# bghira/SimpleTuner

Measured on AMD Instinct MI355X. Metric: training images/sec (whole node), Flux.1-dev LoRA r32 1024^2 train step, higher is better.
Workload: dtype bf16

## Files before the change

### simpletuner_amd/csrc/gemm.hip

```cpp
#include <stdlib.h>
#include <type_traits>
#include "common.h"

#define BK 64
#define EPI_SPLITK 100

#ifdef ST355_TRACE
#define TR_T0 40
#define TR_MARKS 12
__device__ uint64_t st355_trace_buf[2][TR_MARKS];
#define TR_DECL uint64_t tr_[TR_MARKS] = {}
#define TR(t, k)                                                  \
  do {                                                            \
    if ((t) == TR_T0) tr_[k] = __builtin_amdgcn_s_memtime();       \
  } while (0)
#define TR_FLUSH(wv, lane)                                                              \
  do {                                                                                  \
    if (blockIdx.x == 64 && (lane) == 0 && ((wv) & 3) == 0)                              \
      for (int k_ = 0; k_ < TR_MARKS; k_++) st355_trace_buf[(wv) >> 2][k_] = tr_[k_];    \
  } while (0)
#else
#define TR_DECL
#define TR(t, k)
#define TR_FLUSH(wv, lane)
#endif

struct GemmP {
  const bf16* A; int64_t lda;
  const bf16* B; int64_t ldb;
  const bf16* A2; int64_t lda2;
  const bf16* B2; int64_t ldb2;
  bf16* C; int64_t ldc;
  int M, N, K, K2;
  const bf16* bias;
  bf16* aux_out; int64_t ld_aux_out;
  const bf16* aux_in; int64_t ld_aux_in;
  const bf16* gate; int64_t gate_stride; int64_t rows_per_batch;
  float* partial; int ksplit;
  int64_t part_ld;
  const float* scale_a; const float* scale_b;
  int conv_taps, conv_tpt, conv_wp, conv_hp;
  int skip_dead = 1;
  int64_t conv_row0;
  const bf16* img_add; int64_t img_add_stride;
  int seg_rows = 0;
  int64_t seg_xa = 0, seg_xa2 = 0, seg_xc = 0, seg_xin = 0, seg_xout = 0;
  uint32_t tn_magic = 0; int tn_skip_a = 0, tn_skip_b = 0;
  bf16* rq = nullptr; bf16* rk = nullptr; float* rrms = nullptr; bf16* rvt = nullptr; int rSp = 0;
  const bf16* rwq = nullptr; const bf16* rwk = nullptr;
  const float* rcos = nullptr; const float* rsin = nullptr;
  int rH = 0, rS = 0, rpos0 = 0;
  float reps = 0.f;
  int hq = 0, hk = 0;
};

__device__ __forceinline__ GemmP seg_view(const GemmP& p0, int m0) {
  GemmP p = p0;
  if (p0.seg_rows) {
// ... 535 lines not shown
        }
      }
    }
  }
}

__device__ __forceinline__ bool epl_aligned(const GemmP& p) {
  bool ok = (p.N % 8 == 0) && (p.ldc % 8 == 0) && (((uintptr_t)p.C & 15) == 0);
  if (p.bias) ok = ok && (((uintptr_t)p.bias & 15) == 0);
  if (p.aux_out) ok = ok && (p.ld_aux_out % 8 == 0) && (((uintptr_t)p.aux_out & 15) == 0);
  if (p.aux_in) ok = ok && (p.ld_aux_in % 8 == 0) && (((uintptr_t)p.aux_in & 15) == 0);
  if (p.gate) ok = ok && (p.gate_stride % 8 == 0) && (((uintptr_t)p.gate & 15) == 0);
  if (p.img_add) ok = ok && (p.img_add_stride % 8 == 0) && (((uintptr_t)p.img_add & 15) == 0);
  return ok;
}

__device__ __forceinline__ void mma_tile(const char* xs, const char* ws, const int (&x_off)[2], const int (&x_sw)[2],
                                         const int (&w_off)[2], const int (&w_sw)[2], int khalf, f32x16 (&acc)[2][2]) {
#pragma unroll
  for (int ks = 0; ks < 4; ks++) {
    const int c = 2 * ks + khalf;
    bf16x8 wf[2], xf[2];
#pragma unroll
    for (int i = 0; i < 2; i++) {
      wf[i] = *(const bf16x8*)(ws + w_off[i] + ((c ^ w_sw[i]) << 4));
      xf[i] = *(const bf16x8*)(xs + x_off[i] + ((c ^ x_sw[i]) << 4));
    }
#pragma unroll
    for (int i = 0; i < 2; i++)
#pragma unroll
      for (int j = 0; j < 2; j++) acc[i][j] = __builtin_amdgcn_mfma_f32_32x32x16_bf16(wf[i], xf[j], acc[i][j], 0, 0, 0);
  }
}

#define P3_BM 256
#define P3_BN 128
#define P3_THREADS 512
#define P3_XBYTES (P3_BM * BK * 2)
#define P3_WBYTES (P3_BN * BK * 2)
#define P3_STAGE (P3_XBYTES + P3_WBYTES)
#define P3_LDS (3 * P3_STAGE)

template <int EPI>
__global__ void __launch_bounds__(P3_THREADS, 2) k_gemm_p3(GemmGroup g) {
  extern __shared__ __attribute__((aligned(16))) char smem[];
  const int tid = threadIdx.x;
  const int lane = tid & 63;
  const int wv = __builtin_amdgcn_readfirstlane(tid >> 6);
  const int wm = wv >> 1, wn = wv & 1;

  int id = xcd_remap(blockIdx.x, gridDim.x);
  const int pi = id >= g.tiles0 ? 1 : 0;
  if (pi) id -= g.tiles0;
  const GemmP& p0 = g.p[pi];
  const int nbm = (p0.M + P3_BM - 1) / P3_BM, nbn = (p0.N + P3_BN - 1) / P3_BN;
  int pm, pn;
  tile_coords(id, nbm, nbn, pm, pn);
  const int m0 = pm * P3_BM, n0 = pn * P3_BN;
  const GemmP p = seg_view(p0, m0);
  const int nt1 = p.K / BK;
  const int nt = nt1 + p.K2 / BK;

  const bf16* A1 = p.A; const bf16* B1 = p.B; const bf16* A2 = p.A2; const bf16* B2 = p.B2;
  const int64_t la2 = p.lda2, lb2 = p.ldb2;
  const int M = p.M, N = p.N;
  const int st_row = lane >> 3, st_cp = lane & 7;
// ... 2 lines not shown
#pragma unroll
  for (int j = 0; j < 4; j++) {
    const int row = (wv * 4 + j) * 8 + st_row;
    xc[j] = (st_cp ^ ((row >> 1) & 7)) * 8;
    xrow[j] = min(m0 + row, M - 1);
    xo[j] = (int64_t)xrow[j] * p.lda + xc[j];
  }
#pragma unroll
  for (int j = 0; j < 2; j++) {
    const int row = (wv * 2 + j) * 8 + st_row;
    wc[j] = (st_cp ^ ((row >> 1) & 7)) * 8;
    wrow[j] = min(n0 + row, N - 1);
    wo[j] = (int64_t)wrow[j] * p.ldb + wc[j];
  }
  auto stage = [&](int t, int buf) {
    char* xs = smem + buf * P3_STAGE;
    char* ws = xs + P3_XBYTES;
    if (t < nt1) {
      const int k0 = t * BK;
#pragma unroll
      for (int j = 0; j < 4; j++) glds16(A1 + xo[j] + k0, xs + (wv * 4 + j) * 1024);
#pragma unroll
      for (int j = 0; j < 2; j++) glds16(B1 + wo[j] + k0, ws + (wv * 2 + j) * 1024);
    } else {
      const int k0 = (t - nt1) * BK;
#pragma unroll
      for (int j = 0; j < 4; j++) glds16(A2 + (int64_t)xrow[j] * la2 + xc[j] + k0, xs + (wv * 4 + j) * 1024);
#pragma unroll
      for (int j = 0; j < 2; j++) glds16(B2 + (int64_t)wrow[j] * lb2 + wc[j] + k0, ws + (wv * 2 + j) * 1024);
    }
  };

  int w_off[2], w_sw[2], x_off[2], x_sw[2];
#pragma unroll
  for (int i = 0; i < 2; i++) {
    const int wr = wn * 64 + i * 32 + (lane & 31);
    w_off[i] = wr * 128; w_sw[i] = (wr >> 1) & 7;
    const int xr = wm * 64 + i * 32 + (lane & 31);
    x_off[i] = xr * 128; x_sw[i] = (xr >> 1) & 7;
  }
  const int khalf = lane >> 5;
  f32x16 acc[2][2];
#pragma unroll
  for (int i = 0; i < 2; i++)
#pragma unroll
    for (int j = 0; j < 2; j++)
#pragma unroll
      for (int r = 0; r < 16; r++) acc[i][j][r] = 0.f;

  stage(0, 0);
  if (nt > 1) {
    stage(1, 1);
    asm volatile("s_waitcnt vmcnt(6)" ::: "memory");
  } else {
    asm volatile("s_waitcnt vmcnt(0)" ::: "memory");
  }
  __builtin_amdgcn_s_barrier();
  int cur = 0;
  for (int t = 0; t < nt; t++) {
    if (t + 2 < nt) stage(t + 2, cur == 0 ? 2 : cur - 1);
    const char* xs = smem + cur * P3_STAGE;
    mma_tile(xs, xs + P3_XBYTES, x_off, x_sw, w_off, w_sw, khalf, acc);
    if (t + 1 < nt) {
      if (t + 2 < nt) asm volatile("s_waitcnt vmcnt(6)" ::: "memory");
      else asm volatile("s_waitcnt vmcnt(0)" ::: "memory");
      asm volatile("s_waitcnt lgkmcnt(0)" ::: "memory");
      __builtin_amdgcn_s_barrier();
    }
    cur = (cur == 2) ? 0 : cur + 1;
  }
  gemm_epilogue<EPI>(p, acc, m0 + wm * 64, n0 + wn * 64, lane);
}

#define PP_BARRIER()                                   \
  do {                                                 \
    asm volatile("" ::: "memory");                     \
    __builtin_amdgcn_s_barrier();                      \
    asm volatile("" ::: "memory");                     \
  } while (0)

#define PQ_BM 256
#define PQ_BN 256
#define PQ_BK 64
#define PQ_THREADS 512
#define PQ_REGION 16384
#define PQ_BUF (4 * PQ_REGION)
#define PQ_LDS (8 * 64 * 272)
#ifndef PQ_BUFLD
#define PQ_BUFLD 1
#endif
#ifndef PQ_VM
#define PQ_VM 8
#endif
#ifndef PQ_ABL
#define PQ_ABL 0
#endif
#ifndef PQ_PRIO
#ifndef PQ_F8_MX
#define PQ_F8_MX 1
#endif
typedef int i32x8 __attribute__((ext_vector_type(8)));
__device__ __forceinline__ i32x8 frag32(const long* p) {
  i32x8 v;
#pragma unroll
  for (int q = 0; q < 4; q++) { v[2 * q] = (int)(p[q] & 0xffffffffl); v[2 * q + 1] = (int)(p[q] >> 32); }
  return v;
}
#define PQ_PRIO 1
#endif
#ifndef PQ_GL
#define PQ_GL 1
#endif

__device__ __forceinline__ void wait_vm_rt(int n) {
  if (n >= 8) asm volatile("s_waitcnt vmcnt(8)" ::: "memory");
  else if (n == 6) asm volatile("s_waitcnt vmcnt(6)" ::: "memory");
  else if (n == 4) asm volatile("s_waitcnt vmcnt(4)" ::: "memory");
  else if (n == 2) asm volatile("s_waitcnt vmcnt(2)" ::: "memory");
  else asm volatile("s_waitcnt vmcnt(0)" ::: "memory");
}

template <int EPI, bool TN, bool F8 = false, bool CONV = false, int SK = 0>
__global__ void __launch_bounds__(PQ_THREADS, 2) k_gemm_pq(GemmGroup g) {
  static_assert(!SK || (!TN && !F8 && !CONV && EPI != EPI_SPLITK), "the stream-K tail is built for the plain NT bf16 problems");
  constexpr int ES = F8 ? 1 : 2;
  constexpr int KSN = F8 ? 8 : 4;
  static_assert(!(F8 && TN), "fp8 weight gradients are not built");
  extern __shared__ __attribute__((aligned(16))) char smem[];
  const int tid = threadIdx.x;
  const int lane = tid & 63;
  const int wv = __builtin_amdgcn_readfirstlane(tid >> 6);
  const int wm = wv >> 2, wn = wv & 3;

  int slice = (EPI == EPI_SPLITK) ? blockIdx.x / g.tiles0 : 0;
  int id = (EPI == EPI_SPLITK) ? xcd_remap(blockIdx.x % g.tiles0, g.tiles0) : xcd_remap(blockIdx.x, SK ? min((int)gridDim.x, g.sk_first) : (int)gridDim.x);
  int sk_n = 1, sk_tl = 0;
  if (SK && (int)blockIdx.x >= g.sk_first) {
    const int l = blockIdx.x - g.sk_first;
    sk_n = SK;
    const int lq = __builtin_amdgcn_readfirstlane((l >> 3) / sk_n);
    slice = (l >> 3) - lq * sk_n;
    sk_tl = 8 * lq + (l & 7);
    if (sk_tl >= g.tiles0 - g.sk_first) return;
    id = g.sk_first + sk_tl;
  }
  const int pi = id >= g.tiles0 ? 1 : 0;
  if (pi) id -= g.tiles0;
  const GemmP& p = g.p[pi];
  const int nbm = (p.M + PQ_BM - 1) / PQ_BM, nbn = (p.N + PQ_BN - 1) / PQ_BN;
  const int wtaps = (TN && p.conv_taps == 9) ? 9 : 1;
  int pm, pn;
  tile_coords(id, nbm, nbn * wtaps, pm, pn, TN ? ST355_TILE_GROUP : tile_group_for(p.K + p.K2));
  const int wtap = pn / nbn;
  pn -= wtap * nbn;
  const int m0 = pm * PQ_BM, n0 = pn * PQ_BN;
  const int64_t segi = (!TN && !F8 && !CONV && p.seg_rows) ? __builtin_amdgcn_readfirstlane(m0 / p.seg_rows) : 0;
  const int nt_all = p.K / (PQ_BK * 2 / ES);
  const int per = (EPI == EPI_SPLITK) ? (nt_all + p.ksplit - 1) / p.ksplit : SK ? __builtin_amdgcn_readfirstlane((nt_all + sk_n - 1) / sk_n) : nt_all;
  const int t_first = slice * per;
  const int nt1 = (EPI == EPI_SPLITK || SK) ? max(0, min(nt_all, t_first + per) - t_first) : nt_all;
  const int nt = nt1 + ((EPI == EPI_SPLITK || (SK && slice != sk_n - 1)) ? 0 : p.K2 / PQ_BK);
// ... 65 lines not shown
      stage_ext(A2, la2, m0, true, r, (u - nt1) * PQ_BK, dst);
    }
  };
  auto stage_w = [&](int u, int r) {
    char* dst = smem + (u & 1) * PQ_BUF + (2 + r) * PQ_REGION + wv * 2048;
    if (u < nt1) {
      const int w_ko = (int)(u * wk_step) + (TN ? (int)__umulhi((uint32_t)(u + t_first), p.tn_magic) * p.tn_skip_b : 0);
      if (PQ_BUFLD) {
#pragma unroll
        for (int j = 0; j < 2; j++)
          __builtin_amdgcn_raw_ptr_buffer_load_lds(w_rsrc, (__attribute__((address_space(3))) void*)(dst + j * 1024), 16, wo[r][j], w_ko, 0, 0);
        return;
      }
      const char* kb = wbase + w_ko;
#pragma unroll
      for (int j = 0; j < 2; j++) glds16((const bf16*)(kb + wo[r][j]), dst + j * 1024);
    } else {
      stage_ext(B2, lb2, n0, false, r, (u - nt1) * PQ_BK, dst);
    }
  };
  auto refill = [&](int t, int ph, bool check) {
    if (PQ_ABL & 2) return;
    if (ph == 0) { if (!check || t + 1 < nt) stage_w(t + 1, 1); }
    else if (ph == 1) { if (!check || t + 1 < nt) stage_x(t + 1, 1); }
    else if (ph == 2) { if (!check || t + 2 < nt) stage_x(t + 2, 0); }
    else { if (!check || t + 2 < nt) stage_w(t + 2, 0); }
  };

  const int khalf = lane >> 5;
  const int l31 = lane & 31;
  int xk[4], wk[4];
#pragma unroll
  for (int ks = 0; ks < 4; ks++) {
    const int ch = ((2 * ks + khalf) ^ ((l31 >> 1) & 7)) << 4;
    xk[ks] = (wm * 64 + l31) * 128 + ch;
    wk[ks] = 2 * PQ_REGION + (wn * 32 + l31) * 128 + ch;
  }
  const int tg = lane >> 4, tti = (lane >> 2) & 3, tts = lane & 3;
  const int t_row = (8 * (tg >> 1) + tti) * 256 + (tts & 1) * 8;
  const int xt = t_row + (((wm * 8 + 2 * (tg & 1) + (tts >> 1)) ^ (tti << 2)) << 4);
  const int wt = 2 * PQ_REGION + t_row + (((wn * 4 + 2 * (tg & 1) + (tts >> 1)) ^ (tti << 2)) << 4);
  int xk8[8], wk8[8];
#pragma unroll
  for (int ks = 0; ks < 8; ks++) {
    const int chunk = PQ_F8_MX ? 4 * (ks >> 2) + 2 * khalf + ((ks & 3) >> 1) : ks;
    const int half8 = PQ_F8_MX ? (ks & 1) : khalf;
    const int ch = ((chunk ^ ((l31 >> 1) & 7)) << 4) + half8 * 8;
    xk8[ks] = (wm * 64 + l31) * 128 + ch;
    wk8[ks] = 2 * PQ_REGION + (wn * 32 + l31) * 128 + ch;
  }
  auto ld_x8 = [&](const char* base, int j, int ks) -> long { return *(const long*)(base + xk8[ks] + j * 4096); };
  auto ld_w8 = [&](const char* base, int ks) -> long { return *(const long*)(base + wk8[ks]); };
  auto ld_x = [&](const char* base, int j, int ks) -> bf16x8 {
    if (PQ_ABL & 1) { bf16x8 z; for (int q_ = 0; q_ < 8; q_++) z[q_] = (bf16)(float)(lane + j + ks); asm volatile("" : "+v"(z)); return z; }
    if (TN) { const char* q = base + (xt ^ (j << 6)) + ks * 4096; return lds_tr16x2(q, q + 1024); }
    return *(const bf16x8*)(base + xk[ks] + j * 4096);
  };
  auto ld_w = [&](const char* base, int ks) -> bf16x8 {
    if (PQ_ABL & 1) { bf16x8 z; for (int q_ = 0; q_ < 8; q_++) z[q_] = (bf16)(float)(lane + ks); asm volatile("" : "+v"(z)); return z; }
    if (TN) { const char* q = base + wt + ks * 4096; return lds_tr16x2(q, q + 1024); }
    return *(const bf16x8*)(base + wk[ks]);
  };
  f32x16 acc[2][4];
#pragma unroll
  for (int i = 0; i < 2; i++)
#pragma unroll
    for (int j = 0; j < 4; j++)
#pragma unroll
      for (int r = 0; r < 16; r++) acc[i][j][r] = 0.f;

  stage_x(0, 0); stage_w(0, 0); stage_w(0, 1); stage_x(0, 1);
  if (nt > 1) { stage_x(1, 0); stage_w(1, 0); }
  if (PQ_ABL & 2) wait_vm_rt(0); else
  wait_vm_rt(nt > 1 ? 8 : 4);
  PP_BARRIER();
  if (wm == 1) PP_BARRIER();

  bf16x8 xf[2][4], w0f[4], w1f[4];
  long xf8[2][8], w0f8[8], w1f8[8];
  const bool mma_live = !CONV || !p.skip_dead || (n0 + wn * 64 < N);
  TR_DECL;
#define PQ_MMA(WF, I, J0, T, PH)                                                                              \
  do {                                                                                                        \
    if (PQ_PRIO) __builtin_amdgcn_s_setprio(1);                                                               \
    if (F8 && PQ_F8_MX) {                                                                                     \
      _Pragma("unroll") for (int s2 = 0; s2 < 2; s2++)                                                        \
        _Pragma("unroll") for (int j = 0; j < 2; j++)                                                         \
          acc[I][J0 + j] = __builtin_amdgcn_mfma_scale_f32_32x32x64_f8f6f4(frag32(&WF##8[4 * s2]), frag32(&xf8[j][4 * s2]), acc[I][J0 + j], \
                                                                            0 , 1 , 0, 0x7f7f7f7f, 0, 0x7f7f7f7f); \
    } else if (F8) {                                                                                          \
      _Pragma("unroll") for (int ks = 0; ks < 8; ks++)                                                        \
        _Pragma("unroll") for (int j = 0; j < 2; j++)                                                         \
          acc[I][J0 + j] = __builtin_amdgcn_mfma_f32_32x32x16_fp8_bf8(WF##8[ks], xf8[j][ks], acc[I][J0 + j], 0, 0, 0); \
    } else if (!CONV || mma_live)                                                                             \
    _Pragma("unroll") for (int ks = 0; ks < 4; ks++) {                                                        \
      _Pragma("unroll") for (int j = 0; j < 2; j++)                                                           \
        acc[I][J0 + j] = __builtin_amdgcn_mfma_f32_32x32x16_bf16(WF[ks], xf[j][ks], acc[I][J0 + j], 0, 0, 0); \
      if (PQ_GL == 3 && ks == 1) { __builtin_amdgcn_sched_barrier(0); refill(T, PH, TAIL); __builtin_amdgcn_sched_barrier(0); } \
    }                                                                                                         \
    if (PQ_PRIO) __builtin_amdgcn_s_setprio(0);                                                               \
  } while (0)

  auto body = [&](int t, auto tail_c) {
    constexpr bool TAIL = decltype(tail_c)::value;
    const char* bf = smem + (t & 1) * PQ_BUF;
    const int rem = nt - 1 - t;
    TR(t, 0);
    if (PQ_GL == 0) refill(t, 0, TAIL);
#pragma unroll
    for (int j = 0; j < 2; j++)
#pragma unroll
      for (int ks = 0; ks < KSN; ks++) { if (F8) xf8[j][ks] = ld_x8(bf, j, ks); else xf[j][ks & 3] = ld_x(bf, j, ks & 3); }
#pragma unroll
    for (int ks = 0; ks < KSN; ks++) { if (F8) w0f8[ks] = ld_w8(bf, ks); else w0f[ks & 3] = ld_w(bf, ks & 3); }
    if (PQ_GL == 1) refill(t, 0, TAIL);
    TR(t, 1);
    if (!TAIL) wait_vm_rt(PQ_VM); else wait_vm_rt(rem >= 2 ? 8 : (rem == 1 ? 8 : 2));
    PP_BARRIER();
    TR(t, 2);
    PQ_MMA(w0f, 0, 0, t, 1);
    if (PQ_GL == 2) refill(t, 1, TAIL);
    TR(t, 3);
    PP_BARRIER();
    if (PQ_GL == 0) refill(t, 1, TAIL);
#pragma unroll
    for (int ks = 0; ks < KSN; ks++) { if (F8) w1f8[ks] = ld_w8(bf + PQ_REGION, ks); else w1f[ks & 3] = ld_w(bf + PQ_REGION, ks & 3); }
// ... 6 lines not shown
    if (PQ_GL == 2) refill(t, 2, TAIL);
    TR(t, 6);
    PP_BARRIER();
    if (PQ_GL == 0) refill(t, 2, TAIL);
#pragma unroll
    for (int j = 0; j < 2; j++)
#pragma unroll
      for (int ks = 0; ks < KSN; ks++) { if (F8) xf8[j][ks] = ld_x8(bf + PQ_REGION, j, ks); else xf[j][ks & 3] = ld_x(bf + PQ_REGION, j, ks & 3); }
    if (PQ_GL == 1) refill(t, 2, TAIL);
    TR(t, 7);
    if (!TAIL) wait_vm_rt(PQ_VM); else wait_vm_rt(rem >= 2 ? 8 : (rem == 1 ? 6 : 0));
    PP_BARRIER();
    TR(t, 8);
    PQ_MMA(w1f, 1, 2, t, 3);
    if (PQ_GL == 2) refill(t, 3, TAIL);
    TR(t, 9);
    PP_BARRIER();
    if (PQ_GL == 0) refill(t, 3, TAIL);
    if (PQ_GL == 1) refill(t, 3, TAIL);
    if (!TAIL) wait_vm_rt(PQ_VM); else wait_vm_rt(rem >= 2 ? 8 : (rem == 1 ? 4 : 0));
    PP_BARRIER();
    TR(t, 10);
    PQ_MMA(w0f, 0, 2, t + 1, 0);
    if (PQ_GL == 2) refill(t + 1, 0, TAIL);
    TR(t, 11);
    PP_BARRIER();
  };
  if (PQ_GL == 2 || PQ_GL == 3) refill(0, 0, true);
  int t = 0;
  for (; t < nt - 2; t++) body(t, std::false_type{});
  for (; t < nt; t++) body(t, std::true_type{});
#undef PQ_MMA
  TR_FLUSH(wv, lane);
  if (wm == 0) PP_BARRIER();
  if (SK && sk_n > 1) {
    float* slab = g.sk_ws + ((int64_t)sk_tl * (sk_n - 1)) * (PQ_BM * PQ_BN) + tid * 4;
    int* flag = g.sk_flags + sk_tl;
    if (slice < sk_n - 1) {
      slab += (int64_t)slice * (PQ_BM * PQ_BN);
#pragma unroll
      for (int i = 0; i < 2; i++)
#pragma unroll
        for (int j = 0; j < 4; j++)
#pragma unroll
          for (int a = 0; a < 4; a++) {
            f32x4 v;
#pragma unroll
            for (int b = 0; b < 4; b++) v[b] = acc[i][j][4 * a + b];
            *(f32x4*)(slab + ((i * 4 + j) * 4 + a) * (PQ_THREADS * 4)) = v;
          }
      asm volatile("s_waitcnt vmcnt(0)" ::: "memory");
      __syncthreads();
      if (tid == 0) __hip_atomic_fetch_add(flag, 1, __ATOMIC_RELAXED, __HIP_MEMORY_SCOPE_AGENT);
      return;
    }
    if (tid == 0)
      while (__hip_atomic_load(flag, __ATOMIC_RELAXED, __HIP_MEMORY_SCOPE_AGENT) < sk_n - 1) __builtin_amdgcn_s_sleep(4);
    __syncthreads();
    asm volatile("" ::: "memory");
#pragma unroll
    for (int i = 0; i < 2; i++)
#pragma unroll
      for (int j = 0; j < 4; j++) {
        f32x4 v[SK > 1 ? SK - 1 : 1][4];
#pragma unroll
        for (int k = 0; k < SK - 1; k++)
// ... 12 lines not shown
  if (EPI == EPI_SPLITK) {
    GemmP ps = p;
    ps.partial = p.partial + (int64_t)slice * p.M * p.part_ld + (int64_t)wtap * p.N;
    ps.bias = nullptr;
    ps.conv_taps = 0;
    gemm_epilogue_lds<EPI, false, false>(ps, acc, m0 + wm * 128, n0 + wn * 64, lane, smem + wv * EPL_WAVE);
  } else if (wtaps > 1) {
    GemmP ps = p;
    ps.C = p.C + (int64_t)wtap * p.N;
    if (ps.aux_in) ps.aux_in = p.aux_in + (int64_t)wtap * p.N;
    ps.conv_taps = 0;
    gemm_epilogue_lds<EPI, false, false>(ps, acc, m0 + wm * 128, n0 + wn * 64, lane, smem + wv * EPL_WAVE);
  } else if (EPI == ST355_EPI_HEADS) {
    gemm_epilogue_heads(p, p.C + segi * p.seg_xc, acc, m0 + wm * 128, n0 + wn * 64, lane, smem + wv * EPL_WAVE);
  } else if (EPI == ST355_EPI_GEGLU) {
    gemm_epilogue_geglu(p, acc, m0 + wm * 128, n0 + wn * 64, lane, smem + wv * EPL_WAVE);
  } else if (EPI == ST355_EPI_GEGLU_GRAD) {
    gemm_epilogue_geglu_grad(p, acc, m0 + wm * 128, n0 + wn * 64, lane, smem + wv * EPL_WAVE);
  } else if (EPI == ST355_EPI_QK_NORM_ROPE) {
    if (n0 >= 2 * p.rH * 128) {
      gemm_epilogue_vdual(p, p.C + segi * p.seg_xc, acc, m0, n0, wm, wn, wv, lane, smem);
    } else {
      gemm_epilogue_qkrope(p, acc, m0, n0, wm, wn, wv, lane, smem);
    }
  } else if (!TN && !F8 && !CONV) {
    GemmP ps = p;
    ps.C = p.C + segi * p.seg_xc;
    ps.aux_in = p.aux_in + segi * p.seg_xin;
    ps.aux_out = p.aux_out + segi * p.seg_xout;
    if (epl_aligned(ps)) gemm_epilogue_lds<EPI, false, false>(ps, acc, m0 + wm * 128, n0 + wn * 64, lane, smem + wv * EPL_WAVE);
    else gemm_epilogue<EPI, 2, 4>(ps, acc, m0 + wm * 128, n0 + wn * 64, lane);
  } else if (epl_aligned(p)) gemm_epilogue_lds<EPI, CONV, F8>(p, acc, m0 + wm * 128, n0 + wn * 64, lane, smem + wv * EPL_WAVE);
  else gemm_epilogue<EPI, 2, 4>(p, acc, m0 + wm * 128, n0 + wn * 64, lane);
}

#define PZ_LDS (2 * PQ_BUF + 32768)
#define PZ_STAGE 8192

template <int EPI>
__device__ __forceinline__ void gemm_epilogue_lds8(const GemmP& p, f32x16 (&acc)[2][4], int mw0, int nw0, int lane, char* stage) {
  const int khalf = lane >> 5, l31 = lane & 31;
  const int rrow = lane >> 3, rc = lane & 7;
  const int n = nw0 + rc * 8;
  float bias8[8];
#pragma unroll
  for (int b = 0; b < 8; b++) bias8[b] = 0.f;
  if (p.bias) {
    const bf16x8 bv = *(const bf16x8*)(p.bias + n);
#pragma unroll
    for (int b = 0; b < 8; b++) bias8[b] = bf2f(bv[b]);
  }
  const int m_first = mw0 + rrow;
  constexpr bool GG = EPI == ST355_EPI_GEGLU_GRAD;
  const int nc = GG ? 2 * nw0 + 64 * (rc >> 2) + (rc & 3) * 8 : n;
  bf16* c_row = p.C + (int64_t)m_first * p.ldc + nc;
  const bf16* in_row = p.aux_in ? p.aux_in + (int64_t)m_first * p.ld_aux_in + nc : nullptr;
  bf16* out_row = p.aux_out ? p.aux_out + (int64_t)m_first * p.ld_aux_out + n : nullptr;
  const int64_t c_step = 8 * p.ldc, in_step = 8 * p.ld_aux_in, out_step = 8 * p.ld_aux_out;
  typedef __attribute__((address_space(3))) char lds_char;
  typedef __attribute__((address_space(3))) f32x4 lds_f32x4;
  const uint32_t stage_u = (uint32_t)(uintptr_t)(lds_char*)stage;
  const uint32_t wbase0 = stage_u + (uint32_t)(l31 * 256 + ((khalf ^ (l31 & 15)) << 4));
  const uint32_t rb = stage_u + (uint32_t)(rrow * 256);
  const uint32_t r_lo_e = rb + (uint32_t)((((2 * rc) ^ rrow)) << 4), r_hi_e = rb + (uint32_t)((((2 * rc + 1) ^ rrow)) << 4);
  const uint32_t r_lo_o = rb + (uint32_t)((((2 * rc) ^ (rrow | 8))) << 4), r_hi_o = rb + (uint32_t)((((2 * rc + 1) ^ (rrow | 8))) << 4);
  constexpr bool AUXIN = (EPI == ST355_EPI_GATE_RESIDUAL || EPI == ST355_EPI_ADD || EPI == ST355_EPI_MUL_GELU_GRAD || GG);
  bf16x8 auxv[2][4], gatev[2][4];
  const bf16* in_pre = in_row;
  int m_pre = m_first;
  auto preload = [&](bf16x8 (&av)[4], bf16x8 (&gv)[4]) {
#pragma unroll
    for (int it = 0; it < 4; it++) {
      if (AUXIN) av[it] = *(const bf16x8*)in_pre;
      if (EPI == ST355_EPI_GATE_RESIDUAL) gv[it] = *(const bf16x8*)(p.gate + (int64_t)(m_pre / p.rows_per_batch) * p.gate_stride + n);
      if (GG) gv[it] = *(const bf16x8*)(in_pre + 32);
      in_pre += in_step; m_pre += 8;
    }
  };
  if (AUXIN) preload(auxv[0], gatev[0]);
#pragma unroll
  for (int j = 0; j < 4; j++) {
    uint32_t wb = wbase0;
    asm volatile("" : "+v"(wb));
#pragma unroll
    for (int i = 0; i < 2; i++)
#pragma unroll
      for (int a = 0; a < 4; a++) {
        f32x4 v;
#pragma unroll
        for (int b = 0; b < 4; b++) v[b] = acc[i][j][4 * a + b];
        *(lds_f32x4*)(wb ^ (uint32_t)((i * 8 + 2 * a) << 4)) = v;
      }
    if (AUXIN && j < 3) preload(auxv[(j + 1) & 1], gatev[(j + 1) & 1]);
#pragma unroll
    for (int it = 0; it < 4; it++) {
      const f32x4 lo = *(const lds_f32x4*)(((it & 1) ? r_lo_o : r_lo_e) + (uint32_t)(it * 2048));
      const f32x4 hi = *(const lds_f32x4*)(((it & 1) ? r_hi_o : r_hi_e) + (uint32_t)(it * 2048));
      bf16* const c_ptr = c_row;
      bf16* const out_ptr = out_row;
      c_row += c_step; out_row += out_step;
      float v[8];
#pragma unroll
      for (int b = 0; b < 4; b++) { v[b] = lo[b] + bias8[b]; v[4 + b] = hi[b] + bias8[4 + b]; }
      if (EPI == ST355_EPI_GELU) {
        if (p.aux_out) {
          bf16x8 pre;
#pragma unroll
          for (int b = 0; b < 8; b++) pre[b] = f2bf(v[b]);
          *(bf16x8*)out_ptr = pre;
#pragma unroll
          for (int b = 0; b < 8; b++) v[b] = bf2f(pre[b]);
        }
#pragma unroll
        for (int b = 0; b < 8; b++) v[b] = gelu_tanh(v[b]);
      } else if (EPI == ST355_EPI_GATE_RESIDUAL) {
        if (p.aux_out) {
          bf16x8 yv;
#pragma unroll
          for (int b = 0; b < 8; b++) yv[b] = f2bf(v[b]);
          *(bf16x8*)out_ptr = yv;
// ... 6 lines not shown
        const bf16x8 rv = auxv[j & 1][it];
#pragma unroll
        for (int b = 0; b < 8; b++) v[b] += bf2f(rv[b]);
      } else if (EPI == ST355_EPI_MUL_GELU_GRAD) {
        const bf16x8 hv = auxv[j & 1][it];
#pragma unroll
        for (int b = 0; b < 8; b++) v[b] *= gelu_tanh_grad(bf2f(hv[b]));
      }
      if (GG) {
        const bf16x8 vv = auxv[j & 1][it], gv = gatev[j & 1][it];
        bf16x8 dv, dg;
#pragma unroll
        for (int b = 0; b < 8; b++) {
          const float d = bf2f(f2bf(v[b]));
          const float g = bf2f(gv[b]);
          dv[b] = f2bf(d * gelu_erf(g));
          dg[b] = f2bf(d * bf2f(vv[b]) * gelu_erf_grad(g));
        }
        *(bf16x8*)c_ptr = dv;
        *(bf16x8*)(c_ptr + 32) = dg;
        continue;
      }
      bf16x8 o;
#pragma unroll
      for (int b = 0; b < 8; b++) o[b] = f2bf(v[b]);
      *(bf16x8*)c_ptr = o;
    }
  }
}

template <int EPI>
__global__ void __launch_bounds__(PQ_THREADS, 2) k_gemm_pz(GemmP p, int ntiles) {
  extern __shared__ __attribute__((aligned(16))) char smem[];
  const int tid = threadIdx.x;
  const int lane = tid & 63;
  const int wv = __builtin_amdgcn_readfirstlane(tid >> 6);
  const int wm = wv >> 2, wn = wv & 3;
  const int nbm = p.M / PQ_BM, nbn = p.N / PQ_BN;
  const int nt1 = p.K / PQ_BK;
  const int nt = nt1 + p.K2 / PQ_BK;
  const int G = gridDim.x;
  const uint32_t lda_b = (uint32_t)p.lda * 2, ldb_b = (uint32_t)p.ldb * 2;
  const int64_t la2 = p.lda2, lb2 = p.ldb2;

  struct Tile { int m0, n0; const char* xb; const char* wb; const bf16* a2; const bf16* b2; int64_t segi; };
  auto tile_at = [&](int id) {
    Tile t;
    int pm, pn;
    tile_coords(id, nbm, nbn, pm, pn);
    t.m0 = __builtin_amdgcn_readfirstlane(pm * PQ_BM);
    t.n0 = __builtin_amdgcn_readfirstlane(pn * PQ_BN);
    t.segi = p.seg_rows ? (int64_t)__builtin_amdgcn_readfirstlane(t.m0 / p.seg_rows) : 0;
    t.xb = (const char*)(p.A + t.segi * p.seg_xa) + (int64_t)t.m0 * lda_b;
    t.wb = (const char*)p.B + (int64_t)t.n0 * ldb_b;
    t.a2 = p.A2 + t.segi * p.seg_xa2 + (int64_t)t.m0 * la2;
    t.b2 = p.B2 + (int64_t)t.n0 * lb2;
    return t;
  };

  int tile_id = xcd_remap(blockIdx.x, G);
  Tile cur = tile_at(tile_id);
  int par = 0;
  bool first = true;

  while (true) {
    int ln = lane;
    asm volatile("" : "+v"(ln));
    uint32_t xo[2][2], wo[2][2];
#pragma unroll
    for (int j = 0; j < 2; j++) {
      const int lr = (wv * 2 + j) * 8 + (ln >> 3);
      const uint32_t scb = (uint32_t)(((ln & 7) ^ ((lr >> 1) & 7)) * 16);
#pragma unroll
      for (int r = 0; r < 2; r++) {
        xo[r][j] = (uint32_t)((lr >> 6) * 128 + (lr & 63) + r * 64) * lda_b + scb;
        wo[r][j] = (uint32_t)((lr >> 5) * 64 + (lr & 31) + r * 32) * ldb_b + scb;
      }
    }
    const int khalf = ln >> 5;
    const int l31 = ln & 31;
    int xk[4], wk[4];
#pragma unroll
    for (int ks = 0; ks < 4; ks++) {
      const int ch = ((2 * ks + khalf) ^ ((l31 >> 1) & 7)) << 4;
      xk[ks] = (wm * 64 + l31) * 128 + ch;
      wk[ks] = 2 * PQ_REGION + (wn * 32 + l31) * 128 + ch;
    }
    auto ld_x = [&](const char* base, int j, int ks) -> bf16x8 { return *(const bf16x8*)(base + xk[ks] + j * 4096); };
    auto ld_w = [&](const char* base, int ks) -> bf16x8 { return *(const bf16x8*)(base + wk[ks]); };
    const bool has_next = tile_id + G < ntiles;
    const Tile nxt = has_next ? tile_at(tile_id + G) : cur;
    const auto x_rsrc = __builtin_amdgcn_make_buffer_rsrc((void*)cur.xb, 0, 0x7FFFFFFF, 0x00020000);
    const auto w_rsrc = __builtin_amdgcn_make_buffer_rsrc((void*)cur.wb, 0, 0x7FFFFFFF, 0x00020000);
    const auto xn_rsrc = __builtin_amdgcn_make_buffer_rsrc((void*)nxt.xb, 0, 0x7FFFFFFF, 0x00020000);
    const auto wn_rsrc = __builtin_amdgcn_make_buffer_rsrc((void*)nxt.wb, 0, 0x7FFFFFFF, 0x00020000);

    auto stage_x = [&](int u, int r, int mode) {
      char* dst = smem + (((u & 1) ^ par) * PQ_BUF) + r * PQ_REGION + wv * 2048;
      const bool nx = mode == 1 && u >= nt;
      const int uu = nx ? u - nt : u;
      if (uu < nt1) {
#pragma unroll
        for (int j = 0; j < 2; j++)
          __builtin_amdgcn_raw_ptr_buffer_load_lds(nx ? xn_rsrc : x_rsrc, (__attribute__((address_space(3))) void*)(dst + j * 1024), 16, xo[r][j], uu * (PQ_BK * 2), 0, 0);
      } else {
        const bf16* base = nx ? nxt.a2 : cur.a2;
#pragma unroll
        for (int j = 0; j < 2; j++) {
          const int lr = (wv * 2 + j) * 8 + (ln >> 3);
          glds16(base + (int64_t)((lr >> 6) * 128 + (lr & 63) + r * 64) * la2 + ((ln & 7) ^ ((lr >> 1) & 7)) * 8 + (uu - nt1) * PQ_BK, dst + j * 1024);
        }
      }
    };
    auto stage_w = [&](int u, int r, int mode) {
      char* dst = smem + (((u & 1) ^ par) * PQ_BUF) + (2 + r) * PQ_REGION + wv * 2048;
      const bool nx = mode == 1 && u >= nt;
      const int uu = nx ? u - nt : u;
      if (uu < nt1) {
#pragma unroll
        for (int j = 0; j < 2; j++)
          __builtin_amdgcn_raw_ptr_buffer_load_lds(nx ? wn_rsrc : w_rsrc, (__attribute__((address_space(3))) void*)(dst + j * 1024), 16, wo[r][j], uu * (PQ_BK * 2), 0, 0);
      } else {
        const bf16* base = nx ? nxt.b2 : cur.b2;
#pragma unroll
        for (int j = 0; j < 2; j++) {
          const int lr = (wv * 2 + j) * 8 + (ln >> 3);
          glds16(base + (int64_t)((lr >> 5) * 64 + (lr & 31) + r * 32) * lb2 + ((ln & 7) ^ ((lr >> 1) & 7)) * 8 + (uu - nt1) * PQ_BK, dst + j * 1024);
        }
      }
    };
    auto refill = [&](int t, int ph, int mode) {
      const int u = (ph < 2) ? t + 1 : t + 2;
      if (mode == 2 && u >= nt) return;
      if (ph == 0) stage_w(u, 1, mode);
      else if (ph == 1) stage_x(u, 1, mode);
      else if (ph == 2) stage_x(u, 0, mode);
      else stage_w(u, 0, mode);
    };

    f32x16 acc[2][4];
#pragma unroll
    for (int i = 0; i < 2; i++)
#pragma unroll
      for (int j = 0; j < 4; j++)
#pragma unroll
        for (int r = 0; r < 16; r++) acc[i][j][r] = 0.f;

    if (first) {
      stage_x(0, 0, 0); stage_w(0, 0, 0); stage_w(0, 1, 0); stage_x(0, 1, 0);
      stage_x(1, 0, 0); stage_w(1, 0, 0);
      wait_vm_rt(8);
      PP_BARRIER();
    }
    if (wm == 1) PP_BARRIER();

    bf16x8 xf[2][4], w0f[4], w1f[4];
#define PZ_MMA(WF, I, J0)                                                                                     \
  do {                                                                                                        \
    __builtin_amdgcn_s_setprio(1);                                                                            \
    _Pragma("unroll") for (int ks = 0; ks < 4; ks++)                                                          \
      _Pragma("unroll") for (int j = 0; j < 2; j++)                                                           \
        acc[I][J0 + j] = __builtin_amdgcn_mfma_f32_32x32x16_bf16(WF[ks], xf[j][ks], acc[I][J0 + j], 0, 0, 0); \
    __builtin_amdgcn_s_setprio(0);                                                                            \
  } while (0)

    auto body = [&](int t, auto mode_c, auto firstk_c) {
      constexpr int MODE = decltype(mode_c)::value;
      constexpr bool FIRSTK = decltype(firstk_c)::value;
      const char* bf = smem + (((t & 1) ^ par) * PQ_BUF);
      const int rem = nt - 1 - t;
#pragma unroll
      for (int j = 0; j < 2; j++)
#pragma unroll
        for (int ks = 0; ks < 4; ks++) xf[j][ks] = ld_x(bf, j, ks);
#pragma unroll
      for (int ks = 0; ks < 4; ks++) w0f[ks] = ld_w(bf, ks);
      refill(t, 0, MODE);
      if (MODE != 2) { if (!FIRSTK) wait_vm_rt(8); } else wait_vm_rt(rem >= 1 ? 8 : 2);
      PP_BARRIER();
      PZ_MMA(w0f, 0, 0);
      PP_BARRIER();
#pragma unroll
      for (int ks = 0; ks < 4; ks++) w1f[ks] = ld_w(bf + PQ_REGION, ks);
      refill(t, 1, MODE);
      if (MODE != 2) { if (!FIRSTK) wait_vm_rt(8); } else wait_vm_rt(rem >= 1 ? 8 : 0);
      PP_BARRIER();
      PZ_MMA(w1f, 1, 0);
      PP_BARRIER();
#pragma unroll
      for (int j = 0; j < 2; j++)
#pragma unroll
        for (int ks = 0; ks < 4; ks++) xf[j][ks] = ld_x(bf + PQ_REGION, j, ks);
      refill(t, 2, MODE);
      if (MODE != 2) wait_vm_rt(8); else wait_vm_rt(rem >= 1 ? 6 : 0);
      PP_BARRIER();
      PZ_MMA(w1f, 1, 2);
      PP_BARRIER();
      refill(t, 3, MODE);
      if (MODE != 2) wait_vm_rt(8); else wait_vm_rt(rem >= 1 ? 4 : 0);
      PP_BARRIER();
      PZ_MMA(w0f, 0, 2);
      PP_BARRIER();
    };
    int t = 0;
    if (!first) { body(0, std::integral_constant<int, 0>{}, std::true_type{}); t = 1; }
    for (; t < nt - 2; t++) body(t, std::integral_constant<int, 0>{}, std::false_type{});
    for (; t < nt; t++) body(t, std::integral_constant<int, 1>{}, std::false_type{});
#undef PZ_MMA
    if (wm == 0) PP_BARRIER();
    wait_vm_rt(4);
    {
      GemmP ps = p;
      ps.C = p.C + cur.segi * p.seg_xc;
      ps.aux_in = p.aux_in ? p.aux_in + cur.segi * p.seg_xin : nullptr;
      ps.aux_out = p.aux_out ? p.aux_out + cur.segi * p.seg_xout : nullptr;
      char* const lastbuf = smem + ((((nt - 1) & 1) ^ par) * PQ_BUF);
      char* const stg = wv < 2 ? lastbuf + PQ_REGION + wv * PZ_STAGE : (wv < 4 ? lastbuf + 3 * PQ_REGION + (wv - 2) * PZ_STAGE : smem + 2 * PQ_BUF + (wv - 4) * PZ_STAGE);
      int le = lane;
      asm volatile("" : "+v"(le));
      gemm_epilogue_lds8<EPI>(ps, acc, cur.m0 + wm * 128, cur.n0 + wn * 64, le, stg);
    }
    if (!has_next) { wait_vm_rt(0); break; }
    PP_BARRIER();
    par ^= (nt & 1);
    tile_id += G;
    cur = nxt;
    first = false;
  }
}

#define S2_BM 128
#define S2_BN 128
#define S2_THREADS 256
#define S2_TILE (128 * BK * 2)
#define S2_STAGE (2 * S2_TILE)
#define S2_LDS (2 * S2_STAGE)

template <int EPI>
__global__ void __launch_bounds__(S2_THREADS, 2) k_gemm_s2(GemmP p_in) {
  extern __shared__ __attribute__((aligned(16))) char smem[];
  const int tid = threadIdx.x;
  const int lane = tid & 63;
  const int wv = __builtin_amdgcn_readfirstlane(tid >> 6);
  const int wm = wv >> 1, wn = wv & 1;
  const int nbm = (p_in.M + S2_BM - 1) / S2_BM, nbn = (p_in.N + S2_BN - 1) / S2_BN;
  int pm, pn;
  const int tiles = nbm * nbn;
  const int slice = (EPI == EPI_SPLITK) ? blockIdx.x / tiles : 0;
  tile_coords(xcd_remap((EPI == EPI_SPLITK) ? blockIdx.x % tiles : blockIdx.x, tiles), nbm, nbn, pm, pn);
  const int m0 = pm * S2_BM, n0 = pn * S2_BN;
  const GemmP p = seg_view(p_in, m0);
  const int nt1 = p.K / BK;
  const int per = (EPI == EPI_SPLITK) ? (nt1 + p.ksplit - 1) / p.ksplit : 0;
  const int t_first = (EPI == EPI_SPLITK) ? slice * per : 0;
  const int nt = (EPI == EPI_SPLITK) ? min(nt1, t_first + per) : nt1 + p.K2 / BK;
  const int st_row = lane >> 3, st_cp = lane & 7;
  auto stage = [&](int t, int buf) {
    const bf16* Ap; const bf16* Bp; int64_t la, lb; int k0;
    if (t < nt1) { Ap = p.A; la = p.lda; Bp = p.B; lb = p.ldb; k0 = t * BK; }
    else { Ap = p.A2; la = p.lda2; Bp = p.B2; lb = p.ldb2; k0 = (t - nt1) * BK; }
    const int64_t ka = (p.conv_taps && t < nt1) ? conv_koff(p, t, la, BK) : (int64_t)k0;
    char* xs = smem + buf * S2_STAGE;
    char* ws = xs + S2_TILE;
#pragma unroll
    for (int j = 0; j < 4; j++) {
      const int r0 = (wv * 4 + j) * 8;
      const int row = r0 + st_row;
      const int c = st_cp ^ ((row >> 1) & 7);
      glds16(Ap + (int64_t)min(m0 + row, p.M - 1) * la + ka + c * 8, xs + r0 * 128);
      glds16(Bp + (int64_t)min(n0 + row, p.N - 1) * lb + k0 + c * 8, ws + r0 * 128);
    }
  };
  int w_off[2], w_sw[2], x_off[2], x_sw[2];
#pragma unroll
  for (int i = 0; i < 2; i++) {
    const int wr = wn * 64 + i * 32 + (lane & 31);
    w_off[i] = wr * 128; w_sw[i] = (wr >> 1) & 7;
    const int xr = wm * 64 + i * 32 + (lane & 31);
    x_off[i] = xr * 128; x_sw[i] = (xr >> 1) & 7;
  }
  const int khalf = lane >> 5;
  f32x16 acc[2][2];
#pragma unroll
  for (int i = 0; i < 2; i++)
#pragma unroll
    for (int j = 0; j < 2; j++)
#pragma unroll
      for (int r = 0; r < 16; r++) acc[i][j][r] = 0.f;
  if (t_first < nt) stage(t_first, 0);
  __syncthreads();
  for (int t = t_first; t < nt; t++) {
    const int buf = (t - t_first) & 1;
    if (t + 1 < nt) stage(t + 1, buf ^ 1);
    const char* xs = smem + buf * S2_STAGE;
    mma_tile(xs, xs + S2_TILE, x_off, x_sw, w_off, w_sw, khalf, acc);
    __syncthreads();
  }
  if (EPI == EPI_SPLITK) {
    float* slab = p.partial + (int64_t)slice * p.M * p.N;
#pragma unroll
    for (int j = 0; j < 2; j++) {
      const int m = m0 + wm * 64 + j * 32 + (lane & 31);
      if (m >= p.M) continue;
#pragma unroll
      for (int i = 0; i < 2; i++)
#pragma unroll
        for (int a = 0; a < 4; a++) {
          const int n = n0 + wn * 64 + i * 32 + 8 * a + 4 * khalf;
          if (n >= p.N) continue;
          f32x4 v;
#pragma unroll
          for (int b = 0; b < 4; b++) v[b] = acc[i][j][4 * a + b];
          *(f32x4*)(slab + (int64_t)m * p.N + n) = v;
        }
    }
  } else {
    gemm_epilogue<(EPI == EPI_SPLITK) ? ST355_EPI_NONE : EPI>(p, acc, m0 + wm * 64, n0 + wn * 64, lane);
  }
}

__global__ void __launch_bounds__(256) k_splitk_reduce(const float* __restrict__ slabs, int ksplit, const bf16* __restrict__ bias,
                                                      bf16* __restrict__ C, int64_t ldc, int M, int N, int accumulate) {
  const int64_t i4 = (int64_t)blockIdx.x * blockDim.x + threadIdx.x;
  const int n4 = N / 4;
  if (i4 >= (int64_t)M * n4) return;
  const int m = (int)(i4 / n4), n = (int)(i4 % n4) * 4;
  f32x4 s = *(const f32x4*)(slabs + (int64_t)m * N + n);
  for (int k = 1; k < ksplit; k++) {
    const f32x4 v = *(const f32x4*)(slabs + ((int64_t)k * M + m) * N + n);
// ... 896 lines not shown
```

Measured before the change: 6.128.

## Switch bf16 GEMM kernels to 16x16x32 MFMA with permlane accumulator remap

Result: faster. 6.266 (median of 6 runs) (+2.3%).

```diff
diff --git a/simpletuner_amd/csrc/gemm.hip b/simpletuner_amd/csrc/gemm.hip
--- a/simpletuner_amd/csrc/gemm.hip
+++ b/simpletuner_amd/csrc/gemm.hip
@@ -24,6 +24,41 @@
 #define TR(t, k)
 #define TR_FLUSH(wv, lane)
 #endif
+
+#ifdef ST355_CLOCK
+#define CLK_SLOTS 4096
+__device__ uint64_t st355_clock_buf[CLK_SLOTS][2];
+#define CLK_DECL const uint64_t clk_t0_ = __builtin_amdgcn_s_memtime(), clk_r0_ = __builtin_amdgcn_s_memrealtime()
+#define CLK_FLUSH(tid)                                                                                         \
+  do {                                                                                                         \
+    if ((tid) == 0 && blockIdx.x < CLK_SLOTS) {                                                                \
+      const uint64_t t1_ = __builtin_amdgcn_s_memtime(), r1_ = __builtin_amdgcn_s_memrealtime();               \
+      st355_clock_buf[blockIdx.x][0] = t1_ - clk_t0_;                                                          \
+      st355_clock_buf[blockIdx.x][1] = r1_ - clk_r0_;                                                          \
+    }                                                                                                          \
+  } while (0)
+#else
+#define CLK_DECL
+#define CLK_FLUSH(tid)
+#endif
+
+#ifndef PQ_MFMA16
+#define PQ_MFMA16 1
+#endif
+
+__device__ __forceinline__ f32x16 acc16_to_32(const f32x4 (&q)[4]) {
+  f32x16 o;
+#pragma unroll
+  for (int a = 0; a < 2; a++)
+#pragma unroll
+    for (int r = 0; r < 4; r++) {
+      const auto s16 = __builtin_amdgcn_permlane16_swap(__float_as_uint(q[2 * a][r]), __float_as_uint(q[2 * a + 1][r]), false, false);
+      const auto s32 = __builtin_amdgcn_permlane32_swap(s16[0], s16[1], false, false);
+      o[8 * a + r] = __uint_as_float(s32[0]);
+      o[8 * a + 4 + r] = __uint_as_float(s32[1]);
+    }
+  return o;
+}
 
 struct GemmP {
   const bf16* A; int64_t lda;
@@ -625,6 +660,30 @@
       for (int j = 0; j < 2; j++) acc[i][j] = __builtin_amdgcn_mfma_f32_32x32x16_bf16(wf[i], xf[j], acc[i][j], 0, 0, 0);
   }
 }
+__device__ __forceinline__ void mma_tile16(const char* xs, const char* ws, const int (&x_off)[2], const int (&x_sw)[2],
+                                           const int (&w_off)[2], const int (&w_sw)[2], int lane, f32x4 (&acc)[2][2][4]) {
+#pragma unroll
+  for (int s = 0; s < 2; s++) {
+    const int c = 4 * s + (lane >> 4);
+    bf16x8 wf[2][2], xf[2][2];
+#pragma unroll
+    for (int i = 0; i < 2; i++)
+#pragma unroll
+      for (int a = 0; a < 2; a++) {
+        wf[i][a] = *(const bf16x8*)(ws + w_off[i] + a * 2048 + ((c ^ w_sw[i]) << 4));
+        xf[i][a] = *(const bf16x8*)(xs + x_off[i] + a * 2048 + ((c ^ x_sw[i]) << 4));
+      }
+#pragma unroll
+    for (int i = 0; i < 2; i++)
+#pragma unroll
+      for (int a = 0; a < 2; a++)
+#pragma unroll
+        for (int j = 0; j < 2; j++)
+#pragma unroll
+          for (int b = 0; b < 2; b++)
+            acc[i][j][2 * a + b] = __builtin_amdgcn_mfma_f32_16x16x32_bf16(wf[i][a], xf[j][b], acc[i][j][2 * a + b], 0, 0, 0);
+  }
+}
 
 #define P3_BM 256
 #define P3_BN 128
@@ -693,21 +752,26 @@
   };
 
   int w_off[2], w_sw[2], x_off[2], x_sw[2];
+  const int lrow = PQ_MFMA16 ? (lane & 15) : (lane & 31);
 #pragma unroll
   for (int i = 0; i < 2; i++) {
-    const int wr = wn * 64 + i * 32 + (lane & 31);
+    const int wr = wn * 64 + i * 32 + lrow;
     w_off[i] = wr * 128; w_sw[i] = (wr >> 1) & 7;
-    const int xr = wm * 64 + i * 32 + (lane & 31);
+    const int xr = wm * 64 + i * 32 + lrow;
     x_off[i] = xr * 128; x_sw[i] = (xr >> 1) & 7;
   }
   const int khalf = lane >> 5;
   f32x16 acc[2][2];
+  f32x4 acc4[2][2][4];
 #pragma unroll
   for (int i = 0; i < 2; i++)
 #pragma unroll
-    for (int j = 0; j < 2; j++)
+    for (int j = 0; j < 2; j++) {
 #pragma unroll
       for (int r = 0; r < 16; r++) acc[i][j][r] = 0.f;
+#pragma unroll
+      for (int q = 0; q < 4; q++) acc4[i][j][q] = f32x4{0.f, 0.f, 0.f, 0.f};
+    }
 
   stage(0, 0);
   if (nt > 1) {
@@ -721,7 +785,8 @@
   for (int t = 0; t < nt; t++) {
     if (t + 2 < nt) stage(t + 2, cur == 0 ? 2 : cur - 1);
     const char* xs = smem + cur * P3_STAGE;
-    mma_tile(xs, xs + P3_XBYTES, x_off, x_sw, w_off, w_sw, khalf, acc);
+    if (PQ_MFMA16) mma_tile16(xs, xs + P3_XBYTES, x_off, x_sw, w_off, w_sw, lane, acc4);
+    else mma_tile(xs, xs + P3_XBYTES, x_off, x_sw, w_off, w_sw, khalf, acc);
     if (t + 1 < nt) {
       if (t + 2 < nt) asm volatile("s_waitcnt vmcnt(6)" ::: "memory");
       else asm volatile("s_waitcnt vmcnt(0)" ::: "memory");
@@ -729,6 +794,12 @@
       __builtin_amdgcn_s_barrier();
     }
     cur = (cur == 2) ? 0 : cur + 1;
+  }
+  if (PQ_MFMA16) {
+#pragma unroll
+    for (int i = 0; i < 2; i++)
+#pragma unroll
+      for (int j = 0; j < 2; j++) acc[i][j] = acc16_to_32(acc4[i][j]);
   }
   gemm_epilogue<EPI>(p, acc, m0 + wm * 64, n0 + wn * 64, lane);
 }
@@ -786,8 +857,10 @@
   static_assert(!SK || (!TN && !F8 && !CONV && EPI != EPI_SPLITK), "the stream-K tail is built for the plain NT bf16 problems");
   constexpr int ES = F8 ? 1 : 2;
   constexpr int KSN = F8 ? 8 : 4;
+  constexpr bool M16 = PQ_MFMA16 && !TN && !F8;
   static_assert(!(F8 && TN), "fp8 weight gradients are not built");
   extern __shared__ __attribute__((aligned(16))) char smem[];
+  CLK_DECL;
   const int tid = threadIdx.x;
   const int lane = tid & 63;
   const int wv = __builtin_amdgcn_readfirstlane(tid >> 6);
@@ -919,9 +992,10 @@
   int xk[4], wk[4];
 #pragma unroll
   for (int ks = 0; ks < 4; ks++) {
-    const int ch = ((2 * ks + khalf) ^ ((l31 >> 1) & 7)) << 4;
-    xk[ks] = (wm * 64 + l31) * 128 + ch;
-    wk[ks] = 2 * PQ_REGION + (wn * 32 + l31) * 128 + ch;
+    const int rr = M16 ? 16 * (ks >> 1) + (lane & 15) : l31;
+    const int ch = M16 ? ((4 * (ks & 1) + (lane >> 4)) ^ (((lane & 15) >> 1) & 7)) << 4 : ((2 * ks + khalf) ^ ((l31 >> 1) & 7)) << 4;
+    xk[ks] = (wm * 64 + rr) * 128 + ch;
+    wk[ks] = 2 * PQ_REGION + (wn * 32 + rr) * 128 + ch;
   }
   const int tg = lane >> 4, tti = (lane >> 2) & 3, tts = lane & 3;
   const int t_row = (8 * (tg >> 1) + tti) * 256 + (tts & 1) * 8;
@@ -949,12 +1023,16 @@
     return *(const bf16x8*)(base + wk[ks]);
   };
   f32x16 acc[2][4];
+  f32x4 acc4[2][4][4];
 #pragma unroll
   for (int i = 0; i < 2; i++)
 #pragma unroll
-    for (int j = 0; j < 4; j++)
+    for (int j = 0; j < 4; j++) {
 #pragma unroll
       for (int r = 0; r < 16; r++) acc[i][j][r] = 0.f;
+#pragma unroll
+      for (int q = 0; q < 4; q++) acc4[i][j][q] = f32x4{0.f, 0.f, 0.f, 0.f};
+    }
 
   stage_x(0, 0); stage_w(0, 0); stage_w(0, 1); stage_x(0, 1);
   if (nt > 1) { stage_x(1, 0); stage_w(1, 0); }
@@ -979,6 +1057,15 @@
       _Pragma("unroll") for (int ks = 0; ks < 8; ks++)                                                        \
         _Pragma("unroll") for (int j = 0; j < 2; j++)                                                         \
           acc[I][J0 + j] = __builtin_amdgcn_mfma_f32_32x32x16_fp8_bf8(WF##8[ks], xf8[j][ks], acc[I][J0 + j], 0, 0, 0); \
+    } else if (M16) {                                                                                         \
+      if (!CONV || mma_live)                                                                                  \
+      _Pragma("unroll") for (int s = 0; s < 2; s++) {                                                         \
+        _Pragma("unroll") for (int a = 0; a < 2; a++)                                                         \
+          _Pragma("unroll") for (int j = 0; j < 2; j++)                                                       \
+            _Pragma("unroll") for (int b = 0; b < 2; b++)                                                     \
+              acc4[I][J0 + j][2 * a + b] = __builtin_amdgcn_mfma_f32_16x16x32_bf16(WF[2 * a + s], xf[j][2 * b + s], acc4[I][J0 + j][2 * a + b], 0, 0, 0); \
+        if (PQ_GL == 3 && s == 0) { __builtin_amdgcn_sched_barrier(0); refill(T, PH, TAIL); __builtin_amdgcn_sched_barrier(0); } \
+      }                                                                                                       \
     } else if (!CONV || mma_live)                                                                             \
     _Pragma("unroll") for (int ks = 0; ks < 4; ks++) {                                                        \
       _Pragma("unroll") for (int j = 0; j < 2; j++)                                                           \
@@ -1051,6 +1138,12 @@
   for (; t < nt; t++) body(t, std::true_type{});
 #undef PQ_MMA
   TR_FLUSH(wv, lane);
+  if (M16) {
+#pragma unroll
+    for (int i = 0; i < 2; i++)
+#pragma unroll
+      for (int j = 0; j < 4; j++) acc[i][j] = acc16_to_32(acc4[i][j]);
+  }
   if (wm == 0) PP_BARRIER();
   if (SK && sk_n > 1) {
     float* slab = g.sk_ws + ((int64_t)sk_tl * (sk_n - 1)) * (PQ_BM * PQ_BN) + tid * 4;
@@ -1129,13 +1222,14 @@
     else gemm_epilogue<EPI, 2, 4>(ps, acc, m0 + wm * 128, n0 + wn * 64, lane);
   } else if (epl_aligned(p)) gemm_epilogue_lds<EPI, CONV, F8>(p, acc, m0 + wm * 128, n0 + wn * 64, lane, smem + wv * EPL_WAVE);
   else gemm_epilogue<EPI, 2, 4>(p, acc, m0 + wm * 128, n0 + wn * 64, lane);
+  CLK_FLUSH(tid);
 }
 
 #define PZ_LDS (2 * PQ_BUF + 32768)
 #define PZ_STAGE 8192
 
-template <int EPI>
-__device__ __forceinline__ void gemm_epilogue_lds8(const GemmP& p, f32x16 (&acc)[2][4], int mw0, int nw0, int lane, char* stage) {
+template <int EPI, bool Q16 = false>
+__device__ __forceinline__ void gemm_epilogue_lds8(const GemmP& p, f32x16 (&acc)[2][4], const f32x4 (&acc4)[2][4][4], int mw0, int nw0, int lane, char* stage) {
   const int khalf = lane >> 5, l31 = lane & 31;
   const int rrow = lane >> 3, rc = lane & 7;
   const int n = nw0 + rc * 8;
@@ -1157,7 +1251,7 @@
   typedef __attribute__((address_space(3))) char lds_char;
   typedef __attribute__((address_space(3))) f32x4 lds_f32x4;
   const uint32_t stage_u = (uint32_t)(uintptr_t)(lds_char*)stage;
-  const uint32_t wbase0 = stage_u + (uint32_t)(l31 * 256 + ((khalf ^ (l31 & 15)) << 4));
+  const uint32_t wbase0 = Q16 ? stage_u + (uint32_t)((lane & 15) * 256 + (((lane >> 4) ^ (lane & 15)) << 4)) : stage_u + (uint32_t)(l31 * 256 + ((khalf ^ (l31 & 15)) << 4));
   const uint32_t rb = stage_u + (uint32_t)(rrow * 256);
   const uint32_t r_lo_e = rb + (uint32_t)((((2 * rc) ^ rrow)) << 4), r_hi_e = rb + (uint32_t)((((2 * rc + 1) ^ rrow)) << 4);
   const uint32_t r_lo_o = rb + (uint32_t)((((2 * rc) ^ (rrow | 8))) << 4), r_hi_o = rb + (uint32_t)((((2 * rc + 1) ^ (rrow | 8))) << 4);
@@ -1183,6 +1277,10 @@
     for (int i = 0; i < 2; i++)
 #pragma unroll
       for (int a = 0; a < 4; a++) {
+        if (Q16) {
+          *(lds_f32x4*)((wb + (uint32_t)((a & 1) * 4096)) ^ (uint32_t)((i * 8 + 4 * (a >> 1)) << 4)) = acc4[i][j][a];
+          continue;
+        }
         f32x4 v;
 #pragma unroll
         for (int b = 0; b < 4; b++) v[b] = acc[i][j][4 * a + b];
@@ -1255,6 +1353,7 @@
 template <int EPI>
 __global__ void __launch_bounds__(PQ_THREADS, 2) k_gemm_pz(GemmP p, int ntiles) {
   extern __shared__ __attribute__((aligned(16))) char smem[];
+  CLK_DECL;
   const int tid = threadIdx.x;
   const int lane = tid & 63;
   const int wv = __builtin_amdgcn_readfirstlane(tid >> 6);
@@ -1305,9 +1404,10 @@
     int xk[4], wk[4];
 #pragma unroll
     for (int ks = 0; ks < 4; ks++) {
-      const int ch = ((2 * ks + khalf) ^ ((l31 >> 1) & 7)) << 4;
-      xk[ks] = (wm * 64 + l31) * 128 + ch;
-      wk[ks] = 2 * PQ_REGION + (wn * 32 + l31) * 128 + ch;
+      const int rr = PQ_MFMA16 ? 16 * (ks >> 1) + (ln & 15) : l31;
+      const int ch = PQ_MFMA16 ? ((4 * (ks & 1) + (ln >> 4)) ^ (((ln & 15) >> 1) & 7)) << 4 : ((2 * ks + khalf) ^ ((l31 >> 1) & 7)) << 4;
+      xk[ks] = (wm * 64 + rr) * 128 + ch;
+      wk[ks] = 2 * PQ_REGION + (wn * 32 + rr) * 128 + ch;
     }
     auto ld_x = [&](const char* base, int j, int ks) -> bf16x8 { return *(const bf16x8*)(base + xk[ks] + j * 4096); };
     auto ld_w = [&](const char* base, int ks) -> bf16x8 { return *(const bf16x8*)(base + wk[ks]); };
@@ -1362,12 +1462,16 @@
     };
 
     f32x16 acc[2][4];
+    f32x4 acc4[2][4][4];
 #pragma unroll
     for (int i = 0; i < 2; i++)
 #pragma unroll
-      for (int j = 0; j < 4; j++)
+      for (int j = 0; j < 4; j++) {
 #pragma unroll
         for (int r = 0; r < 16; r++) acc[i][j][r] = 0.f;
+#pragma unroll
+        for (int q = 0; q < 4; q++) acc4[i][j][q] = f32x4{0.f, 0.f, 0.f, 0.f};
+      }
 
     if (first) {
       stage_x(0, 0, 0); stage_w(0, 0, 0); stage_w(0, 1, 0); stage_x(0, 1, 0);
@@ -1381,9 +1485,17 @@
 #define PZ_MMA(WF, I, J0)                                                                                     \
   do {                                                                                                        \
     __builtin_amdgcn_s_setprio(1);                                                                            \
-    _Pragma("unroll") for (int ks = 0; ks < 4; ks++)                                                          \
-      _Pragma("unroll") for (int j = 0; j < 2; j++)                                                           \
-        acc[I][J0 + j] = __builtin_amdgcn_mfma_f32_32x32x16_bf16(WF[ks], xf[j][ks], acc[I][J0 + j], 0, 0, 0); \
+    if (PQ_MFMA16) {                                                                                          \
+      _Pragma("unroll") for (int s = 0; s < 2; s++)                                                           \
+        _Pragma("unroll") for (int a = 0; a < 2; a++)                                                         \
+          _Pragma("unroll") for (int j = 0; j < 2; j++)                                                       \
+            _Pragma("unroll") for (int b = 0; b < 2; b++)                                                     \
+              acc4[I][J0 + j][2 * a + b] = __builtin_amdgcn_mfma_f32_16x16x32_bf16(WF[2 * a + s], xf[j][2 * b + s], acc4[I][J0 + j][2 * a + b], 0, 0, 0); \
+    } else {                                                                                                  \
+      _Pragma("unroll") for (int ks = 0; ks < 4; ks++)                                                        \
+        _Pragma("unroll") for (int j = 0; j < 2; j++)                                                         \
+          acc[I][J0 + j] = __builtin_amdgcn_mfma_f32_32x32x16_bf16(WF[ks], xf[j][ks], acc[I][J0 + j], 0, 0, 0); \
+    }                                                                                                         \
     __builtin_amdgcn_s_setprio(0);                                                                            \
   } while (0)
 
@@ -1441,9 +1553,9 @@
       char* const stg = wv < 2 ? lastbuf + PQ_REGION + wv * PZ_STAGE : (wv < 4 ? lastbuf + 3 * PQ_REGION + (wv - 2) * PZ_STAGE : smem + 2 * PQ_BUF + (wv - 4) * PZ_STAGE);
       int le = lane;
       asm volatile("" : "+v"(le));
-      gemm_epilogue_lds8<EPI>(ps, acc, cur.m0 + wm * 128, cur.n0 + wn * 64, le, stg);
-    }
-    if (!has_next) { wait_vm_rt(0); break; }
+      gemm_epilogue_lds8<EPI, PQ_MFMA16>(ps, acc, acc4, cur.m0 + wm * 128, cur.n0 + wn * 64, le, stg);
+    }
+    if (!has_next) { wait_vm_rt(0); CLK_FLUSH(tid); break; }
     PP_BARRIER();
     par ^= (nt & 1);
     tile_id += G;
@@ -1495,29 +1607,41 @@
     }
   };
   int w_off[2], w_sw[2], x_off[2], x_sw[2];
+  const int lrow = PQ_MFMA16 ? (lane & 15) : (lane & 31);
 #pragma unroll
   for (int i = 0; i < 2; i++) {
-    const int wr = wn * 64 + i * 32 + (lane & 31);
+    const int wr = wn * 64 + i * 32 + lrow;
     w_off[i] = wr * 128; w_sw[i] = (wr >> 1) & 7;
-    const int xr = wm * 64 + i * 32 + (lane & 31);
+    const int xr = wm * 64 + i * 32 + lrow;
     x_off[i] = xr * 128; x_sw[i] = (xr >> 1) & 7;
   }
   const int khalf = lane >> 5;
   f32x16 acc[2][2];
+  f32x4 acc4[2][2][4];
 #pragma unroll
   for (int i = 0; i < 2; i++)
 #pragma unroll
-    for (int j = 0; j < 2; j++)
+    for (int j = 0; j < 2; j++) {
 #pragma unroll
       for (int r = 0; r < 16; r++) acc[i][j][r] = 0.f;
+#pragma unroll
+      for (int q = 0; q < 4; q++) acc4[i][j][q] = f32x4{0.f, 0.f, 0.f, 0.f};
+    }
   if (t_first < nt) stage(t_first, 0);
   __syncthreads();
   for (int t = t_first; t < nt; t++) {
     const int buf = (t - t_first) & 1;
     if (t + 1 < nt) stage(t + 1, buf ^ 1);
     const char* xs = smem + buf * S2_STAGE;
-    mma_tile(xs, xs + S2_TILE, x_off, x_sw, w_off, w_sw, khalf, acc);
+    if (PQ_MFMA16) mma_tile16(xs, xs + S2_TILE, x_off, x_sw, w_off, w_sw, lane, acc4);
+    else mma_tile(xs, xs + S2_TILE, x_off, x_sw, w_off, w_sw, khalf, acc);
     __syncthreads();
+  }
+  if (PQ_MFMA16) {
+#pragma unroll
+    for (int i = 0; i < 2; i++)
+#pragma unroll
+      for (int j = 0; j < 2; j++) acc[i][j] = acc16_to_32(acc4[i][j]);
   }
   if (EPI == EPI_SPLITK) {
     float* slab = p.partial + (int64_t)slice * p.M * p.N;
```
